# cts198859/deeprl_signal_control

Measured on NVIDIA H100. Metric: agent-env-steps/sec, higher is better.
Workload: dtype f32 (sim, LSTM cell, loss, optimizer) + bf16 tensor-core operands with f32 accumulation (learner GEMMs)

## Files before the change

### deeprl_signal_control_b200/_lib.py

```python
from __future__ import annotations

import ctypes as C
import os
import subprocess

_HERE = os.path.dirname(os.path.abspath(__file__))
CSRC = os.path.join(_HERE, "csrc")
LIB_PATH = os.environ.get("TSC_LIB", os.path.join(CSRC, "libtsc.so"))
_lib = None

SYMBOLS = ["tsc_last_error", "tsc_create", "tsc_destroy", "tsc_reset", "tsc_set_train_mode",
           "tsc_observe", "tsc_step", "tsc_step_host", "tsc_step_host_range", "tsc_step_host_range_async", "tsc_set_record", "tsc_step_record", "tsc_get_trips", "tsc_get_counts", "tsc_get_traffic_stats",
           "tsc_dump_state", "tsc_info", "tsc_mean_live", "tsc_set_greedy_program", "tsc_greedy_actions",
           "tscl_create", "tscl_destroy", "tscl_fc_embed", "tscl_lstm_seq_fwd", "tscl_heads", "tscl_returns",
           "tscl_heads_loss", "tscl_lstm_seq_bwd", "tscl_fc_bwd", "tscl_fc_bwd_tc", "tscl_wgrad_tc", "tscl_clip_rmsprop",
           "tscl_pack_weights", "tscl_policy_step", "tscl_policy_step_v2", "tscl_policy_step_v2r", "tscl_unpack_store", "tscl_pack_wht", "tscl_lstm_seq_bwd_tc", "tscl_pack_wxt", "tscl_lstm_seq_bwd_tc_dx", "tscl_dx_tc", "tscl_host_transition", "tscl_device_transition", "tscl_memcpy_async", "tscl_fc_hidden_fwd", "tscl_fc_hidden_bwd", "tscl_debug_policy_prof", "tscl_debug_bptt_prof",
           "tscl_policy_step_pi", "tscl_argmax_actions", "tscl_q_create", "tscl_q_destroy", "tscl_q_step",
           "tscl_q_explore", "tscl_q_sample", "tscl_q_td", "tscl_q_adam", "tscl_q_transition"]


def build_native(force: bool = False, verbose: bool = False) -> str:
    cmd = ["make", "-C", CSRC] + (["-B"] if force else [])
    out = subprocess.run(cmd, capture_output=True, text=True)
    if out.returncode != 0:
        raise RuntimeError("nvcc build of libtsc.so failed:\n" + out.stdout + out.stderr)
    if verbose:
        print(out.stdout + out.stderr)
    return LIB_PATH


def lib() -> C.CDLL:
    global _lib
    if _lib is None:
        if not os.path.exists(LIB_PATH):
            raise ImportError(
                "native library %s is missing: run `python -c 'import __graft_entry__ as g; g.build()'` "
                "(there is no CPU fallback)" % LIB_PATH)
        _lib = C.CDLL(LIB_PATH)
        _lib.tsc_last_error.restype = C.c_char_p
        for s in SYMBOLS:
            getattr(_lib, s)
    return _lib


def check(rc: int):
    if rc != 0:
        raise RuntimeError("libtsc: " + lib().tsc_last_error().decode())
```

### deeprl_signal_control_b200/agents/learner.py

```python
from __future__ import annotations

import ctypes as C
import os
from typing import Optional

import numpy as np
import torch

from .. import _lib
from .. import dist as _dist
from .layout import PolicyLayout


def _p(t):
    return None if t is None else C.c_void_p(t.data_ptr())


class BatchedA2C:
    def __init__(self, layout: PolicyLayout, n_replicas: int, n_step: int, gamma: float = 0.99,
                 v_coef: float = 0.5, max_grad_norm: float = 40.0, alpha: float = 0.99, eps: float = 1e-5,
                 reward_norm: float = 1.0, reward_clip: float = 0.0, seed: int = 0, device: int = 0,
                 chunk: int = 1024, replica0: int = 0, total_replicas: Optional[int] = None,
                 process_group=None, allow_tf32: bool = True, use_tc: bool = True,
                 store_acts: Optional[bool] = None):
# ... 27 lines not shown
        self.c_bw = torch.zeros_like(self.c_fw); self.h_bw = torch.zeros_like(self.h_fw)
        self.c_tmp = torch.zeros_like(self.c_fw); self.h_tmp = torch.zeros_like(self.h_fw)
        self.X1 = torch.empty(U, R, L.dx, **f32)
        self.Z1 = torch.empty(U, R, 4 * L.h, **f32)
        self.H1 = torch.empty(U, R, L.h, **f32)
        self.pi = torch.zeros(R, A, L.max_na, **f32)
        self.val = torch.zeros(R, A, **f32)
        self.act = torch.zeros(R, A, dtype=torch.int32, device=self.dev)
        self.boot = torch.zeros(R, A, **f32)
        self.obs_hist = torch.zeros(T + 1, R, L.n_obs, **f32)
        self.act_hist = torch.zeros(T, R, A, dtype=torch.int32, device=self.dev)
        self.rew_hist = torch.zeros(T, R, A, **f32)
        self.val_hist = torch.zeros(T, R, A, **f32)
        self.Rs = torch.zeros(T, R, A, **f32); self.Adv = torch.zeros(T, R, A, **f32)
        self.done_pre = [0.0] * T
        self.done_post = [0.0] * T
        self.last_done = False
        self.t = 0
        self.n_forward = 0
        self._one = torch.zeros(1, **f32)
        self._upd_bufs = None
        self.kernel_launches = 0
        self.use_tc = bool(use_tc) and (L.dx % 16 == 0) and layout.kw > 0
        if self.use_tc and L.dx > 224:
            raise ValueError("the tensor-core policy forward supports dx <= 224 (got %d); use use_tc=False" % L.dx)
        self.tc_v2 = self.use_tc and L.dx in (160, 192, 224)
        self.Wp = torch.zeros(U, ((L.dx + L.h) // 8) * 4 * L.h * 8 + 8 * L.dx * 8, dtype=torch.bfloat16,
                              device=self.dev)
        self.Wt = torch.zeros(U, 32, L.h, 8, dtype=torch.bfloat16, device=self.dev)
        self.Wxt = torch.zeros(U, 32, L.dx, 8, dtype=torch.bfloat16, device=self.dev)
        self.dx_fused = False
        self.dx_fusable = self.use_tc and L.dx % 32 == 0 and L.dx <= 256
        self.dx_own = self.use_tc and L.dx % 16 == 0 and L.dx <= 224 and os.environ.get("TSC_DX_LIBRARY", "0") != "1"
        self.bwd_tc = self.use_tc
        self.fc_bwd_tc = self.use_tc and layout.fc_bwd_tc_ok
        self.wgrad_tc = self.use_tc and L.dx % 8 == 0 and L.dx <= 240
        self.fused_heads = True
        self.pack_weights()
        need = U * T * R * (L.dx + 4 * L.h + 2 * L.h) * 2
        if store_acts is None:
            free, _ = torch.cuda.mem_get_info(self.dev)
            store_acts = self.tc_v2 and need < 0.5 * free
        self.store_acts = bool(store_acts) and self.tc_v2 and (R % self.chunk == 0)
        self.st_x = self.st_g = self.st_c = self.st_h = None
        if self.store_acts:
            bf = dict(dtype=torch.bfloat16, device=self.dev)
            nc, rc_ = R // self.chunk, self.chunk
            self.st_x = torch.zeros(nc, U, T, rc_, L.dx, **bf); self.st_g = torch.zeros(nc, U, T, rc_, 4 * L.h, **bf)
            self.st_c = torch.zeros(nc, U, T, rc_, L.h, **bf); self.st_h = torch.zeros(nc, U, T, rc_, L.h, **bf)
        self._acts_ok = [False] * T

    def close(self):
        if getattr(self, "_h", None) is not None:
            _lib.lib().tscl_destroy(self._h)
            self._h = None

    def __del__(self):
        try:
            self.close()
        except Exception:
            pass

    def _st(self):
        return C.c_void_p(torch.cuda.current_stream(self.dev).cuda_stream)

    def pack_weights(self):
# ... 97 lines not shown
        self.t += 1

    def obs_slot(self, t: Optional[int] = None) -> torch.Tensor:
        return self.obs_hist[self.t if t is None else t]

    def add_transition(self, reward: torch.Tensor, done_pre: bool, done_post: bool,
                       act: Optional[torch.Tensor] = None, val: Optional[torch.Tensor] = None):
        t = self.t
        r = reward
        if self.reward_norm:
            r = r / self.reward_norm
        if self.reward_clip:
            r = torch.clamp(r, -self.reward_clip, self.reward_clip)
        self.rew_hist[t].copy_(r)
        self.act_hist[t].copy_(self.act if act is None else act)
        self.val_hist[t].copy_(self.val if val is None else val)
        self.done_pre[t] = 1.0 if done_pre else 0.0
        self.done_post[t] = 1.0 if done_post else 0.0
        self.t += 1

    def add_transition_device(self, reward: torch.Tensor, greward: torch.Tensor, rew_acc: torch.Tensor, done_pre: bool,
                              done_post: bool):
        t = self.t
        _lib.check(_lib.lib().tscl_device_transition(
            self._h, _p(reward), _p(self.rew_hist[t]), C.c_int64(reward.numel()), C.c_float(self.reward_norm or 0.0),
            C.c_float(self.reward_clip or 0.0), _p(greward), _p(rew_acc), C.c_int64(greward.numel()), self._st()))
        if not getattr(self, "_hist_direct", False):
            self.act_hist[t].copy_(self.act)
            self.val_hist[t].copy_(self.val)
        self.done_pre[t] = 1.0 if done_pre else 0.0
        self.done_post[t] = 1.0 if done_post else 0.0
        self.t += 1

    def _bufs(self, rc, lean=False):
        L, T, U = self.lay, self.T, self.lay.U
        f32 = dict(dtype=torch.float32, device=self.dev)
        if self._upd_bufs is None or self._upd_bufs["rc"] < rc:
            M = T * rc
            self._upd_bufs = dict(rc=rc, dH=torch.empty(U, M, L.h, **f32))
        b = self._upd_bufs
        M = T * b["rc"]
        if lean and "dZb" not in b:
            b.update(dZb=torch.empty(U, M, 4 * L.h, dtype=torch.bfloat16, device=self.dev),
                     dXb=torch.empty(U, M, L.dx, dtype=torch.bfloat16, device=self.dev))
        if not lean and "X" not in b:
            b.update(ZG=torch.empty(U, M, 4 * L.h, **f32), dX=torch.empty(U, M, L.dx, **f32),
                     X=torch.empty(U, M, L.dx, **f32), C=torch.empty(U, M, L.h, **f32), H=torch.empty(U, M, L.h, **f32),
                     Hp=torch.empty(U, M, L.h, **f32), dlog=torch.empty(U, M, L.max_na, **f32))
        return b

    def backward(self, boot: Optional[torch.Tensor], lr: float, beta: float):
        assert self.t == self.T, "rollout buffer not full"
        L, R, T, U, A, lib = self.lay, self.R, self.T, self.lay.U, self.lay.A, _lib.lib()
        self._mm()
        st = self._st
        f32 = dict(dtype=torch.float32, device=self.dev)
        dpre = torch.tensor(self.done_pre, **f32)
        dpost = torch.tensor(self.done_post, **f32)
        if boot is None:
            self.boot.zero_()
        else:
            self.boot.copy_(boot)
        _lib.check(lib.tscl_returns(self._h, _p(self.rew_hist), _p(self.val_hist), _p(self.boot), _p(dpost),
                                    C.c_float(self.gamma), C.c_int32(T), C.c_int64(R), _p(self.Rs), _p(self.Adv), st()))
        self.G.zero_()
        self.stats.zero_()
        scale = _dist.grad_scale(T, 1, self.total_replicas)
        use_store = self.store_acts and all(self._acts_ok)
        n_obs = L.n_obs
        for r0 in range(0, R, self.chunk):
            rc = min(self.chunk, R - r0)
            M = T * rc
            ci = r0 // self.chunk
            all_tc = use_store and self.bwd_tc and self.fc_bwd_tc and self.wgrad_tc and self.fused_heads
            b = self._bufs(rc, lean=all_tc)
            X = Cc = H = Hp = dlog = ZG = dX = dZb = dXb = None
            bf16 = dict(dtype=torch.bfloat16, device=self.dev)
            if b["rc"] == rc:
                dH = b["dH"]
                if all_tc:
                    dZb, dXb = b["dZb"], b["dXb"]
                else:
                    ZG, dX, X, Cc, H, Hp, dlog = (b[k] for k in ("ZG", "dX", "X", "C", "H", "Hp", "dlog"))
            else:
                dH = torch.empty(U, M, L.h, **f32)
                if all_tc:
                    dZb, dXb = torch.empty(U, M, 4 * L.h, **bf16), torch.empty(U, M, L.dx, **bf16)
                else:
                    ZG, dX, X, Cc, H, Hp, dlog = (torch.empty(U, M, s_, **f32) for s_ in
                                                  (4 * L.h, L.dx, L.dx, L.h, L.h, L.h, L.max_na))
            obs0 = self.obs_hist[0, r0:]
            if all_tc:
                pass
            elif use_store:
                direct = self.bwd_tc
                _lib.check(lib.tscl_unpack_store(self._h, _p(self.st_x[ci]), _p(self.st_g[ci]), _p(self.st_c[ci]),
                                                 _p(self.st_h[ci]), _p(X), None if direct else _p(ZG),
                                                 None if direct else _p(Cc), _p(H), _p(Hp), _p(self.h_bw),
                                                 _p(dpre), C.c_int32(T), C.c_int64(rc), C.c_int64(R), C.c_int64(r0),
                                                 st()))
            else:
                _lib.check(lib.tscl_fc_embed(self._h, _p(self.P), _p(obs0), C.c_int64(M), C.c_int64(rc),
                                             C.c_int64(R * n_obs), _p(X), st()))
                torch.baddbmm(self.pv["bl"].unsqueeze(1), X, self.pv["wx"], out=ZG)
                _lib.check(lib.tscl_lstm_seq_fwd(self._h, _p(self.P), _p(ZG), _p(Cc), _p(H), _p(Hp), _p(self.c_bw),
                                                 _p(self.h_bw), None, None, _p(dpre), C.c_int32(T), C.c_int64(rc),
                                                 C.c_int64(R), C.c_int64(r0), st()))
            hb = _p(self.st_h[ci]) if use_store else None
            _lib.check(lib.tscl_heads_loss(self._h, _p(self.P), None if all_tc else _p(H), _p(self.act_hist[0, r0:]),
                                           _p(self.Rs[0, r0:]), _p(self.Adv[0, r0:]), C.c_int64(M), C.c_int64(rc),
                                           C.c_int64(R * A), C.c_float(self.v_coef), C.c_float(beta), C.c_float(scale),
                                           None if self.fused_heads else _p(dlog), _p(dH), _p(self.stats),
                                           hb if all_tc else None, _p(self.G) if self.fused_heads else None, st()))
            if not self.fused_heads:
                self.gv["wo"].baddbmm_(H.transpose(1, 2), dlog)
                self.gv["bo"].add_(dlog.sum(dim=1))
            fuse_dx = all_tc and self.dx_fused and self.dx_fusable
            if self.bwd_tc:
                gb = (_p(self.st_g[ci]), _p(self.st_c[ci])) if use_store else (None, None)
                _lib.check(lib.tscl_lstm_seq_bwd_tc_dx(self._h, _p(self.Wt), _p(ZG), _p(Cc), _p(dH), _p(self.c_bw),
                                                       _p(dpre), C.c_int32(T), C.c_int64(rc), C.c_int64(R), C.c_int64(r0),
                                                       *gb, _p(dZb), _p(self.Wxt) if fuse_dx else None,
                                                       _p(dXb) if fuse_dx else None, st()))
            else:
                _lib.check(lib.tscl_lstm_seq_bwd(self._h, _p(self.P), _p(ZG), _p(Cc), _p(dH), _p(self.c_bw), _p(dpre),
                                                 C.c_int32(T), C.c_int64(rc), C.c_int64(R), C.c_int64(r0), st()))
            dZ = ZG
            if self.wgrad_tc:
                if use_store:
                    _lib.check(lib.tscl_wgrad_tc(self._h, _p(dZ), _p(dZb), None, _p(self.st_x[ci]), None, _p(self.st_h[ci]),
                                                 _p(self.h_bw), _p(dpre), C.c_int32(T), C.c_int64(rc), C.c_int64(R),
                                                 C.c_int64(r0), _p(self.G), C.c_int32(0), st()))
                else:
                    _lib.check(lib.tscl_wgrad_tc(self._h, _p(dZ), None, _p(X), None, _p(Hp), None, None, None, C.c_int32(T),
                                                 C.c_int64(rc), C.c_int64(R), C.c_int64(r0), _p(self.G), C.c_int32(0), st()))
            else:
                self.gv["wx"].baddbmm_(X.transpose(1, 2), dZ)
                self.gv["wh"].baddbmm_(Hp.transpose(1, 2), dZ)
                self.gv["bl"].add_(dZ.sum(dim=1))
            if all_tc and not fuse_dx and self.dx_own:
                _lib.check(lib.tscl_dx_tc(self._h, _p(dZb), _p(self.Wxt), _p(dXb), C.c_int64(M), st()))
            elif all_tc and not fuse_dx:
                torch.bmm(dZb, self.wx_b.transpose(1, 2), out=dXb)
            elif not all_tc:
                torch.bmm(dZ, self.pv["wx"].transpose(1, 2), out=dX)
            if self.fc_bwd_tc:
                xb = _p(self.st_x[ci]) if use_store else None
                _lib.check(lib.tscl_fc_bwd_tc(self._h, _p(obs0), None if all_tc else _p(X), xb, _p(dX), _p(dXb),
                                              C.c_int64(M), C.c_int64(rc), C.c_int64(R * n_obs), _p(self.G), C.c_int32(0),
                                              st()))
            else:
                _lib.check(lib.tscl_fc_bwd(self._h, _p(obs0), _p(X), _p(dX), C.c_int64(M), C.c_int64(rc),
                                           C.c_int64(R * n_obs), _p(self.G), st()))
            self.kernel_launches += 4 if use_store else 5
        if self.pg is not None:
            _dist.allreduce_sum_(self.G, self.pg)
        _lib.check(lib.tscl_clip_rmsprop(self._h, _p(self.P), _p(self.G), _p(self.MS), _p(self.agent_of),
                                         C.c_float(self.max_grad_norm), C.c_float(lr), C.c_float(self.alpha),
                                         C.c_float(self.eps), _p(self.norms), st()))
        self.kernel_launches += 3
        self.pack_weights()
        self.c_bw.copy_(self.c_fw); self.h_bw.copy_(self.h_fw)
        self.obs_hist[0].copy_(self.obs_hist[T])
        self.last_done = bool(self.done_post[-1])
        self.t = 0
        self._acts_ok = [False] * T
```

### deeprl_signal_control_b200/csrc/tsc_policy_tc.cu

```cuda
#include <cuda.h>
#include <cstdlib>
#include <cuda_bf16.h>
#include <cuda_runtime.h>
#include <stdint.h>

#include <string>

#include "../../include/tsc_learn.h"

int tsc_set_error(const std::string& m);
#define PCK(call)                                                                  \
  do {                                                                             \
    cudaError_t e__ = (call);                                                      \
    if (e__ != cudaSuccess) return tsc_set_error(std::string(#call) + ": " + cudaGetErrorString(e__)); \
  } while (0)

struct DDimsTC {
  int A, n_obs, max_na, fw, ff, ft, h, dx;
  const int32_t *obs_off, *n_wave, *n_wait, *n_fp, *n_a;
  const int64_t *off_fcw_w, *off_fcw_b, *off_fcf_w, *off_fcf_b, *off_fct_w, *off_fct_b;
  int64_t off_wx, off_wh, off_bl, off_wo, off_bo, n_params;
  int kw, ones_slot;
};
const DDimsTC* tscl_dims_of(tscl_handle* h);
// ... 1363 lines not shown
      wg_fence();
#pragma unroll
      for (int g = 0; g < 4; ++g)
#pragma unroll
        for (int c = 0; c < 4; ++c)
          wgmma_n64_rs(acc, af[g][2 * c][0], af[g][2 * c][1], af[g][2 * c + 1][0], af[g][2 * c + 1][1],
                       make_desc(aB + (4 * g + c) * 2 * 1024, 1024, 128), (g | c) != 0);
      wg_commit();
      BR_MARK(2);
      asm volatile("bar.sync %0, 128;" ::"r"(1 + wg) : "memory");
      if (lead) {
#pragma unroll
        for (int g = 0; g < 4; ++g) tma_store_3d(&mapZ, g * 64, rw0, z0 + t, aZ + g * 8192);
        asm volatile("cp.async.bulk.commit_group;" ::: "memory");
      }
      BR_MARK(3);
      wg_wait<0>();
      wg_frag_fence(acc);
      const bool need_dh = keep != 0.f && t > 0;
#pragma unroll
      for (int j = 0; j < 8; ++j)
#pragma unroll
        for (int e = 0; e < 4; ++e) dhc[j][e] = need_dh ? acc[4 * j + e] * keep : 0.f;
      BR_MARK(2);
    }
  }
  if (lead) asm volatile("cp.async.bulk.wait_group 0;" ::: "memory");
  if (PROF && lead)
    for (int i = 0; i < 4; ++i) atomicAdd(a.prof + i, (unsigned long long)bp[i]);
#undef BR_MARK
}

static bool make_tmap_3d(CUtensorMap* m, CUtensorMapDataType dt, int elem_bytes, const void* base, uint64_t planes,
                         uint64_t rows, uint64_t cols, uint32_t box_cols, uint32_t box_rows) {
  typedef CUresult (*encode_fn)(CUtensorMap*, CUtensorMapDataType, cuuint32_t, void*, const cuuint64_t*, const cuuint64_t*,
                                const cuuint32_t*, const cuuint32_t*, CUtensorMapInterleave, CUtensorMapSwizzle,
                                CUtensorMapL2promotion, CUtensorMapFloatOOBfill);
  static encode_fn fn = []() -> encode_fn {
    void* p = nullptr;
    cudaDriverEntryPointQueryResult q;
    if (cudaGetDriverEntryPoint("cuTensorMapEncodeTiled", &p, cudaEnableDefault, &q) != cudaSuccess || q != cudaDriverEntryPointSuccess)
      return nullptr;
    return (encode_fn)p;
  }();
  if (!fn || !base) return false;
  memset(m, 0, sizeof(*m));
  const cuuint64_t dims[3] = {cols, rows, planes};
  const cuuint64_t strides[2] = {cols * (uint64_t)elem_bytes, rows * cols * (uint64_t)elem_bytes};
  const cuuint32_t box[3] = {box_cols, box_rows, 1};
  const cuuint32_t es[3] = {1, 1, 1};
  return fn(m, dt, 3, const_cast<void*>(base), dims, strides, box, es, CU_TENSOR_MAP_INTERLEAVE_NONE, CU_TENSOR_MAP_SWIZZLE_128B,
            CU_TENSOR_MAP_L2_PROMOTION_L2_128B, CU_TENSOR_MAP_FLOAT_OOB_FILL_NONE) == CUDA_SUCCESS;
}

__device__ __forceinline__ void cp_async16(uint32_t dst, const void* src) {
  asm volatile("cp.async.cg.shared.global [%0], [%1], 16;" ::"r"(dst), "l"(src) : "memory");
}

extern "C" int tscl_pack_wxt(tscl_handle* h, const float* params, void* wxt_bf16, void* stream) {
  if (!h || !params || !wxt_bf16) return tsc_set_error("tscl_pack_wxt: bad argument");
  PCK(cudaSetDevice(tscl_device_of(h)));
  const DDimsTC& d = *tscl_dims_of(h);
  pack_wxt_kernel<<<dim3(8, 2 * d.A), 256, 0, (cudaStream_t)stream>>>(d, params, (__nv_bfloat16*)wxt_bf16);
  PCK(cudaGetLastError());
  return 0;
}

extern "C" int tscl_pack_wht(tscl_handle* h, const float* params, void* wt_bf16, void* stream) {
  if (!h || !params || !wt_bf16) return tsc_set_error("tscl_pack_wht: bad argument");
  PCK(cudaSetDevice(tscl_device_of(h)));
  const DDimsTC& d = *tscl_dims_of(h);
  pack_wht_kernel<<<dim3(2, 2 * d.A), 256, 0, (cudaStream_t)stream>>>(d, params, (__nv_bfloat16*)wt_bf16);
  PCK(cudaGetLastError());
  return 0;
}

extern "C" int tscl_lstm_seq_bwd_tc(tscl_handle* h, const void* wt_bf16, float* ZG, const float* C, const float* dH,
                                    const float* c0, const float* done, int32_t T, int64_t Rc, int64_t ld_state,
                                    int64_t r0, const void* gates_bf16, const void* c_bf16, void* dz_bf16, void* stream) {
  return tscl_lstm_seq_bwd_tc_dx(h, wt_bf16, ZG, C, dH, c0, done, T, Rc, ld_state, r0, gates_bf16, c_bf16, dz_bf16, nullptr,
                                 nullptr, stream);
}

extern "C" int tscl_lstm_seq_bwd_tc_dx(tscl_handle* h, const void* wt_bf16, float* ZG, const float* C, const float* dH,
// ... 853 lines not shown
  __syncthreads();
}

extern "C" int tscl_dx_tc(tscl_handle* h, const void* dz_bf16, const void* wxt_bf16, void* dx_bf16, int64_t M, void* stream) {
  if (!h || !dz_bf16 || !wxt_bf16 || !dx_bf16 || M <= 0) return tsc_set_error("tscl_dx_tc: bad argument");
  PCK(cudaSetDevice(tscl_device_of(h)));
  const DDimsTC& d = *tscl_dims_of(h);
  if (d.dx % 16 != 0 || d.dx > 224 || d.dx < 16) return tsc_set_error("tscl_dx_tc: dx must be a multiple of 16 in [16, 224]");
  const size_t smem = (size_t)DXK_STAGES * DXK_STAGE_BYTES + (size_t)BW_KC * d.dx * 16 + (size_t)128 * (d.dx * 2 + 16) + 12 * 8 + 16;
  if (smem > 232448) return tsc_set_error("tscl_dx_tc: shared memory budget exceeded");
  void (*kern)(const DDimsTC, const DxTC) = nullptr;
  switch (d.dx) {
#define DXK_CASE(n) case n: kern = dx_tc_kernel<n>; break;
    DXK_CASE(16) DXK_CASE(32) DXK_CASE(48) DXK_CASE(64) DXK_CASE(80) DXK_CASE(96) DXK_CASE(112) DXK_CASE(128)
    DXK_CASE(144) DXK_CASE(160) DXK_CASE(176) DXK_CASE(192) DXK_CASE(208) DXK_CASE(224)
#undef DXK_CASE
  }
  static int attr_dev = -1;
  static void (*attr_kern)(const DDimsTC, const DxTC) = nullptr;
  if (attr_dev != tscl_device_of(h) || attr_kern != kern) {
    PCK(cudaFuncSetAttribute(kern, cudaFuncAttributeMaxDynamicSharedMemorySize, 232448));
    attr_dev = tscl_device_of(h); attr_kern = kern;
  }
  int n_sm = 0;
  PCK(cudaDeviceGetAttribute(&n_sm, cudaDevAttrMultiProcessorCount, tscl_device_of(h)));
  const int64_t NT = ((M + 127) / 128) * 2 * d.A;
  const int grid = (int)(NT < n_sm ? NT : n_sm);
  DxTC a;
  a.dZb = (const __nv_bfloat16*)dz_bf16; a.Wxt = (const __nv_bfloat16*)wxt_bf16; a.dXb = (__nv_bfloat16*)dx_bf16; a.M = M;
  kern<<<grid, DXK_THREADS, smem, (cudaStream_t)stream>>>(d, a);
  PCK(cudaGetLastError());
  return 0;
}
```

### include/tsc_learn.h

```cpp
#ifndef TSC_LEARN_H_
#define TSC_LEARN_H_

#include <stdint.h>

#ifdef __cplusplus
extern "C" {
#endif

typedef struct tscl_dims {
  int32_t n_agents;
  int32_t n_obs;
  int32_t max_na;
  int32_t fw, ff, ft;
  int32_t h;
  int32_t dx;
  const int32_t* obs_off;
  const int32_t* n_wave;
  const int32_t* n_wait;
  const int32_t* n_fp;
  const int32_t* n_a;
  const int64_t* off_fcw_w;  const int64_t* off_fcw_b;
  const int64_t* off_fcf_w;  const int64_t* off_fcf_b;
  const int64_t* off_fct_w;  const int64_t* off_fct_b;
  int64_t off_wx;
// ... 32 lines not shown
                    void* stream);

int tscl_lstm_seq_bwd(tscl_handle* h, const float* params, float* ZG, const float* C, const float* dH,
                      const float* c0, const float* done, int32_t T, int64_t Rc, int64_t ld_state, int64_t r0,
                      void* stream);

int tscl_fc_bwd(tscl_handle* h, const float* obs, const float* X, const float* dX, int64_t M,
                int64_t rows_per_t, int64_t stride_t, float* grads, void* stream);

int tscl_fc_bwd_tc(tscl_handle* h, const float* obs, const float* X, const void* x_bf16, const float* dX,
                   const void* dx_bf16, int64_t M, int64_t rows_per_t, int64_t stride_t, float* grads, int32_t variant,
                   void* stream);

int tscl_wgrad_tc(tscl_handle* h, const float* dZ, const void* dz_bf16, const float* X, const void* x_bf16,
                  const float* Hp, const void* h_bf16, const float* h0, const float* done, int32_t T, int64_t rc,
                  int64_t ld_state, int64_t r0, float* grads, int32_t variant, void* stream);

int tscl_pack_wht(tscl_handle* h, const float* params, void* wt_bf16, void* stream);
int tscl_lstm_seq_bwd_tc(tscl_handle* h, const void* wt_bf16, float* ZG, const float* C, const float* dH, const float* c0,
                         const float* done, int32_t T, int64_t Rc, int64_t ld_state, int64_t r0,
                         const void* gates_bf16, const void* c_bf16, void* dz_bf16, void* stream);
int tscl_pack_wxt(tscl_handle* h, const float* params, void* wxt_bf16, void* stream);
int tscl_lstm_seq_bwd_tc_dx(tscl_handle* h, const void* wt_bf16, float* ZG, const float* C, const float* dH, const float* c0,
                            const float* done, int32_t T, int64_t Rc, int64_t ld_state, int64_t r0,
                            const void* gates_bf16, const void* c_bf16, void* dz_bf16, const void* wxt_bf16, void* dx_bf16,
                            void* stream);
int tscl_host_transition(tscl_handle* h, const float* obs_host, float* obs_dev, int64_t obs_floats, const float* rew_host,
                         float* rew_stage_dev, float* rew_hist_dev, int64_t rew_floats, float reward_norm, float reward_clip,
                         const float* grew_host, float* grew_stage_dev, float* rew_acc_dev, int64_t n, void* stream);
int tscl_device_transition(tscl_handle* h, const float* rew_dev, float* rew_hist_dev, int64_t rew_floats, float reward_norm,
                           float reward_clip, const float* grew_dev, float* rew_acc_dev, int64_t n, void* stream);
int tscl_memcpy_async(tscl_handle* h, void* dst, const void* src, int64_t bytes, int32_t kind, void* stream);
int tscl_dx_tc(tscl_handle* h, const void* dz_bf16, const void* wxt_bf16, void* dx_bf16, int64_t M, void* stream);

int tscl_unpack_store(tscl_handle* h, const void* st_x, const void* st_g, const void* st_c, const void* st_h, float* X,
                      float* ZG, float* C, float* H, float* Hp, const float* h0, const float* done, int32_t T,
                      int64_t rc, int64_t ld_state, int64_t r0, void* stream);

int tscl_debug_policy_prof(void* counters_dev);
int tscl_debug_bptt_prof(void* counters_dev);

int tscl_clip_rmsprop(tscl_handle* h, float* params, float* grads, float* ms, const uint8_t* agent_of,
                      float max_norm, float lr, float alpha, float eps, float* norms, void* stream);

int tscl_pack_weights(tscl_handle* h, const float* params, void* wpack_bf16, void* stream);
int tscl_policy_step(tscl_handle* h, const float* params, const void* wpack_bf16, const float* obs, int64_t R,
                     const float* c_in, const float* h_in, float* c_out, float* h_out, float* pi, float* val,
                     int32_t* act, int32_t done, uint64_t seed, int64_t step, int64_t replica0, float* zdbg,
                     int32_t swap_lbo_sbo, void* stream);

int tscl_policy_step_v2(tscl_handle* h, const float* params, const void* wpack_bf16, const float* obs, int64_t R,
                        const float* c_in, const float* h_in, float* c_out, float* h_out, float* pi, float* val,
                        int32_t* act, int32_t done, uint64_t seed, int64_t step, int64_t replica0, float* zdbg,
                        void* st_x, void* st_g, void* st_c, void* st_h, int32_t t, int32_t T, int64_t rc, void* stream);
int tscl_policy_step_v2r(tscl_handle* h, const float* params, const void* wpack_bf16, const float* obs, int64_t R,
                         const float* c_in, const float* h_in, float* c_out, float* h_out, float* pi, float* val,
                         int32_t* act, int32_t done, uint64_t seed, int64_t step, int64_t replica0, float* zdbg,
                         void* st_x, void* st_g, void* st_c, void* st_h, int32_t t, int32_t T, int64_t rc,
                         int64_t ld_state, int64_t row0, void* stream);
int tscl_policy_step_pi(tscl_handle* h, const float* params, const void* wpack_bf16, const float* obs, int64_t R,
                        const float* c_in, const float* h_in, float* c_out, float* h_out, float* pi, int32_t* act,
                        int32_t act_mode, int32_t done, uint64_t seed, int64_t step, int64_t replica0, int64_t ld_state,
                        int64_t row0, void* stream);
int tscl_argmax_actions(tscl_handle* h, const float* pi, int64_t R, int32_t* act, void* stream);

typedef struct tscl_qdims {
// ... 40 lines not shown
```

Baseline: 22.59 million.

## Fuse LSTM input-gradient GEMM with FC-embedding weight-gradient backward kernel

Adds a warp-specialized Hopper kernel that computes dX = dZ·Wx^T with wgmma. It applies the ReLU mask from the stored activations in shared memory and immediately uses the masked dX tile for the FC weight-gradient GEMM against observations gathered on the fly. This removes the bf16 dX round trip through global memory and one kernel launch per chunk. In exchange it brings register-split setmaxnreg, TMA pipelines and atomic gradient flushes, limited to dx in {160,192,224}.

```diff
diff --git a/deeprl_signal_control_b200/_lib.py b/deeprl_signal_control_b200/_lib.py
--- a/deeprl_signal_control_b200/_lib.py
+++ b/deeprl_signal_control_b200/_lib.py
@@ -14,7 +14,7 @@
            "tsc_dump_state", "tsc_info", "tsc_mean_live", "tsc_set_greedy_program", "tsc_greedy_actions",
            "tscl_create", "tscl_destroy", "tscl_fc_embed", "tscl_lstm_seq_fwd", "tscl_heads", "tscl_returns",
            "tscl_heads_loss", "tscl_lstm_seq_bwd", "tscl_fc_bwd", "tscl_fc_bwd_tc", "tscl_wgrad_tc", "tscl_clip_rmsprop",
-           "tscl_pack_weights", "tscl_policy_step", "tscl_policy_step_v2", "tscl_policy_step_v2r", "tscl_unpack_store", "tscl_pack_wht", "tscl_lstm_seq_bwd_tc", "tscl_pack_wxt", "tscl_lstm_seq_bwd_tc_dx", "tscl_dx_tc", "tscl_host_transition", "tscl_device_transition", "tscl_memcpy_async", "tscl_fc_hidden_fwd", "tscl_fc_hidden_bwd", "tscl_debug_policy_prof", "tscl_debug_bptt_prof",
+           "tscl_pack_weights", "tscl_policy_step", "tscl_policy_step_v2", "tscl_policy_step_v2r", "tscl_unpack_store", "tscl_pack_wht", "tscl_lstm_seq_bwd_tc", "tscl_pack_wxt", "tscl_lstm_seq_bwd_tc_dx", "tscl_dx_tc", "tscl_dx_fc_bwd_tc", "tscl_host_transition", "tscl_device_transition", "tscl_memcpy_async", "tscl_fc_hidden_fwd", "tscl_fc_hidden_bwd", "tscl_debug_policy_prof", "tscl_debug_bptt_prof",
            "tscl_policy_step_pi", "tscl_argmax_actions", "tscl_q_create", "tscl_q_destroy", "tscl_q_step",
            "tscl_q_explore", "tscl_q_sample", "tscl_q_td", "tscl_q_adam", "tscl_q_transition"]
 
diff --git a/deeprl_signal_control_b200/agents/learner.py b/deeprl_signal_control_b200/agents/learner.py
--- a/deeprl_signal_control_b200/agents/learner.py
+++ b/deeprl_signal_control_b200/agents/learner.py
@@ -83,6 +83,7 @@
         self.dx_fused = False
         self.dx_fusable = self.use_tc and L.dx % 32 == 0 and L.dx <= 256
         self.dx_own = self.use_tc and L.dx % 16 == 0 and L.dx <= 224 and os.environ.get("TSC_DX_LIBRARY", "0") != "1"
+        self.dx_fc_fused = self.dx_own and self.tc_v2
         self.bwd_tc = self.use_tc
         self.fc_bwd_tc = self.use_tc and layout.fc_bwd_tc_ok
         self.wgrad_tc = self.use_tc and L.dx % 8 == 0 and L.dx <= 240
@@ -246,7 +247,7 @@
         self.done_post[t] = 1.0 if done_post else 0.0
         self.t += 1
 
-    def _bufs(self, rc, lean=False):
+    def _bufs(self, rc, lean=False, dxb=True):
         L, T, U = self.lay, self.T, self.lay.U
         f32 = dict(dtype=torch.float32, device=self.dev)
         if self._upd_bufs is None or self._upd_bufs["rc"] < rc:
@@ -255,8 +256,9 @@
         b = self._upd_bufs
         M = T * b["rc"]
         if lean and "dZb" not in b:
-            b.update(dZb=torch.empty(U, M, 4 * L.h, dtype=torch.bfloat16, device=self.dev),
-                     dXb=torch.empty(U, M, L.dx, dtype=torch.bfloat16, device=self.dev))
+            b["dZb"] = torch.empty(U, M, 4 * L.h, dtype=torch.bfloat16, device=self.dev)
+        if lean and dxb and "dXb" not in b:
+            b["dXb"] = torch.empty(U, M, L.dx, dtype=torch.bfloat16, device=self.dev)
         if not lean and "X" not in b:
             b.update(ZG=torch.empty(U, M, 4 * L.h, **f32), dX=torch.empty(U, M, L.dx, **f32),
                      X=torch.empty(U, M, L.dx, **f32), C=torch.empty(U, M, L.h, **f32), H=torch.empty(U, M, L.h, **f32),
@@ -287,19 +289,22 @@
             M = T * rc
             ci = r0 // self.chunk
             all_tc = use_store and self.bwd_tc and self.fc_bwd_tc and self.wgrad_tc and self.fused_heads
-            b = self._bufs(rc, lean=all_tc)
+            fuse_dx = all_tc and self.dx_fused and self.dx_fusable
+            fuse_fc = all_tc and not fuse_dx and self.dx_fc_fused
+            b = self._bufs(rc, lean=all_tc, dxb=not fuse_fc)
             X = Cc = H = Hp = dlog = ZG = dX = dZb = dXb = None
             bf16 = dict(dtype=torch.bfloat16, device=self.dev)
             if b["rc"] == rc:
                 dH = b["dH"]
                 if all_tc:
-                    dZb, dXb = b["dZb"], b["dXb"]
+                    dZb, dXb = b["dZb"], b.get("dXb")
                 else:
                     ZG, dX, X, Cc, H, Hp, dlog = (b[k] for k in ("ZG", "dX", "X", "C", "H", "Hp", "dlog"))
             else:
                 dH = torch.empty(U, M, L.h, **f32)
                 if all_tc:
-                    dZb, dXb = torch.empty(U, M, 4 * L.h, **bf16), torch.empty(U, M, L.dx, **bf16)
+                    dZb = torch.empty(U, M, 4 * L.h, **bf16)
+                    dXb = None if fuse_fc else torch.empty(U, M, L.dx, **bf16)
                 else:
                     ZG, dX, X, Cc, H, Hp, dlog = (torch.empty(U, M, s_, **f32) for s_ in
                                                   (4 * L.h, L.dx, L.dx, L.h, L.h, L.h, L.max_na))
@@ -329,7 +334,6 @@
             if not self.fused_heads:
                 self.gv["wo"].baddbmm_(H.transpose(1, 2), dlog)
                 self.gv["bo"].add_(dlog.sum(dim=1))
-            fuse_dx = all_tc and self.dx_fused and self.dx_fusable
             if self.bwd_tc:
                 gb = (_p(self.st_g[ci]), _p(self.st_c[ci])) if use_store else (None, None)
                 _lib.check(lib.tscl_lstm_seq_bwd_tc_dx(self._h, _p(self.Wt), _p(ZG), _p(Cc), _p(dH), _p(self.c_bw),
@@ -352,13 +356,18 @@
                 self.gv["wx"].baddbmm_(X.transpose(1, 2), dZ)
                 self.gv["wh"].baddbmm_(Hp.transpose(1, 2), dZ)
                 self.gv["bl"].add_(dZ.sum(dim=1))
-            if all_tc and not fuse_dx and self.dx_own:
+            if fuse_fc:
+                _lib.check(lib.tscl_dx_fc_bwd_tc(self._h, _p(obs0), _p(self.st_x[ci]), _p(dZb), _p(self.Wxt), C.c_int64(M),
+                                                 C.c_int64(rc), C.c_int64(R * n_obs), _p(self.G), st()))
+            elif all_tc and not fuse_dx and self.dx_own:
                 _lib.check(lib.tscl_dx_tc(self._h, _p(dZb), _p(self.Wxt), _p(dXb), C.c_int64(M), st()))
             elif all_tc and not fuse_dx:
                 torch.bmm(dZb, self.wx_b.transpose(1, 2), out=dXb)
             elif not all_tc:
                 torch.bmm(dZ, self.pv["wx"].transpose(1, 2), out=dX)
-            if self.fc_bwd_tc:
+            if fuse_fc:
+                pass
+            elif self.fc_bwd_tc:
                 xb = _p(self.st_x[ci]) if use_store else None
                 _lib.check(lib.tscl_fc_bwd_tc(self._h, _p(obs0), None if all_tc else _p(X), xb, _p(dX), _p(dXb),
                                               C.c_int64(M), C.c_int64(rc), C.c_int64(R * n_obs), _p(self.G), C.c_int32(0),
@@ -366,7 +375,7 @@
             else:
                 _lib.check(lib.tscl_fc_bwd(self._h, _p(obs0), _p(X), _p(dX), C.c_int64(M), C.c_int64(rc),
                                            C.c_int64(R * n_obs), _p(self.G), st()))
-            self.kernel_launches += 4 if use_store else 5
+            self.kernel_launches += 3 if fuse_fc else 4 if use_store else 5
         if self.pg is not None:
             _dist.allreduce_sum_(self.G, self.pg)
         _lib.check(lib.tscl_clip_rmsprop(self._h, _p(self.P), _p(self.G), _p(self.MS), _p(self.agent_of),
diff --git a/deeprl_signal_control_b200/csrc/tsc_policy_tc.cu b/deeprl_signal_control_b200/csrc/tsc_policy_tc.cu
--- a/deeprl_signal_control_b200/csrc/tsc_policy_tc.cu
+++ b/deeprl_signal_control_b200/csrc/tsc_policy_tc.cu
@@ -1419,7 +1419,8 @@
 }
 
 static bool make_tmap_3d(CUtensorMap* m, CUtensorMapDataType dt, int elem_bytes, const void* base, uint64_t planes,
-                         uint64_t rows, uint64_t cols, uint32_t box_cols, uint32_t box_rows) {
+                         uint64_t rows, uint64_t cols, uint32_t box_cols, uint32_t box_rows,
+                         CUtensorMapSwizzle sw = CU_TENSOR_MAP_SWIZZLE_128B) {
   typedef CUresult (*encode_fn)(CUtensorMap*, CUtensorMapDataType, cuuint32_t, void*, const cuuint64_t*, const cuuint64_t*,
                                 const cuuint32_t*, const cuuint32_t*, CUtensorMapInterleave, CUtensorMapSwizzle,
                                 CUtensorMapL2promotion, CUtensorMapFloatOOBfill);
@@ -1436,7 +1437,7 @@
   const cuuint64_t strides[2] = {cols * (uint64_t)elem_bytes, rows * cols * (uint64_t)elem_bytes};
   const cuuint32_t box[3] = {box_cols, box_rows, 1};
   const cuuint32_t es[3] = {1, 1, 1};
-  return fn(m, dt, 3, const_cast<void*>(base), dims, strides, box, es, CU_TENSOR_MAP_INTERLEAVE_NONE, CU_TENSOR_MAP_SWIZZLE_128B,
+  return fn(m, dt, 3, const_cast<void*>(base), dims, strides, box, es, CU_TENSOR_MAP_INTERLEAVE_NONE, sw,
             CU_TENSOR_MAP_L2_PROMOTION_L2_128B, CU_TENSOR_MAP_FLOAT_OOB_FILL_NONE) == CUDA_SUCCESS;
 }
 
@@ -2356,3 +2357,321 @@
   PCK(cudaGetLastError());
   return 0;
 }
+
+#define DXF_THREADS 384
+#define DXF_STAGES 2
+#define DXF_SBO 2048
+#define DXF_BUILDERS 96
+#define DXF_CONS_REGS(dx) ((dx) > 192 ? 216 : 208)
+#define DXF_PROD_REGS(dx) ((dx) > 192 ? 72 : 80)
+static_assert(128 * DXF_PROD_REGS(224) + 256 * DXF_CONS_REGS(224) <= DXF_THREADS * 168 &&
+              128 * DXF_PROD_REGS(160) + 256 * DXF_CONS_REGS(160) <= DXF_THREADS * 168,
+              "setmaxnreg split exceeds the CTA's registers");
+static size_t dxf_smem(int dx) {
+  return (size_t)DXF_STAGES * DXK_STAGE_BYTES + (size_t)BW_KC * dx * 16 + (size_t)(dx / 8) * DXF_SBO + 8 * FBT_SBO + 8 * 8;
+}
+struct DxFcTC {
+  const float* obs;
+  const __nv_bfloat16* Wxt;
+  float* G;
+  int64_t M, rows_per_t, stride_t;
+};
+__device__ __forceinline__ uint32_t bf16x2_pos_mask(uint32_t x) {
+  const uint32_t nz = ((x & 0x7FFF7FFFu) + 0x7FFF7FFFu) & ~x & 0x80008000u;
+  return (nz >> 15) * 0xFFFFu;
+}
+template <int NR>
+__device__ __forceinline__ void dxf_flush(const DDimsTC& d, float* G, int u, const float (&f)[NR], int cb) {
+  const int lane = threadIdx.x & 31, w4 = (threadIdx.x >> 5) & 3, ag = u >> 1;
+  const int nw = d.n_wave[ag], nt = d.n_wait[ag], nf = d.ff > 0 ? d.n_fp[ag] : 0;
+#pragma unroll
+  for (int e = 0; e < NR; ++e) {
+    const int slot = 16 * w4 + (lane >> 2) + 8 * ((e >> 1) & 1);
+    const int c = cb + 8 * (e >> 2) + 2 * (lane & 3) + (e & 1);
+    int64_t wo, bo; int ld, cc, s0, n;
+    if (c < d.fw) { wo = d.off_fcw_w[u]; bo = d.off_fcw_b[u]; ld = d.fw; cc = c; s0 = 0; n = nw; }
+    else if (c < d.fw + d.ff) { wo = d.off_fcf_w[u]; bo = d.off_fcf_b[u]; ld = d.ff; cc = c - d.fw; s0 = d.kw; n = nf; }
+    else { wo = d.off_fct_w[u]; bo = d.off_fct_b[u]; ld = d.ft; cc = c - d.fw - d.ff; s0 = d.kw + TC_KF; n = nt; }
+    const int kin = slot - s0;
+    if (kin >= 0 && kin < n) atomicAdd(&G[wo + (int64_t)kin * ld + cc], f[e]);
+    if (slot == d.ones_slot) atomicAdd(&G[bo + cc], f[e]);
+  }
+}
+
+template <int DX>
+__global__ void __launch_bounds__(DXF_THREADS, 1)
+dx_fc_bwd_tc_kernel(const DDimsTC d, const DxFcTC a, const __grid_constant__ CUtensorMap mapZ,
+                    const __grid_constant__ CUtensorMap mapX) {
+  constexpr int N64 = DX / 64, R32 = (DX % 64) >= 32, R16 = (DX % 32) >= 16;
+  constexpr int HN = DX / 2, H32 = (HN % 64) >= 32, H16 = (HN % 32) >= 16;
+  static_assert(HN >= 64 && HN < 128 && HN % 16 == 0, "fc half width must be 64 + {0, 16, 32, 48}");
+  const int tid = threadIdx.x, warp = tid >> 5, lane = tid & 31;
+  unsigned char* sStage = tc_smem;
+  unsigned char* sW = sStage + DXF_STAGES * DXK_STAGE_BYTES;
+  unsigned char* sA = sW + (size_t)BW_KC * DX * 16;
+  unsigned char* sB = sA + (size_t)(DX / 8) * DXF_SBO;
+  uint64_t* sBar = reinterpret_cast<uint64_t*>(sB + 8 * FBT_SBO);
+  const uint32_t bar_full = smem_u32(sBar), bar_empty = bar_full + 16, bar_w = bar_full + 32, bar_x = bar_full + 40,
+                 bar_in = bar_full + 48, bar_free = bar_full + 56;
+  if (tid == 0) {
+    for (int s = 0; s < DXF_STAGES; ++s) { mbar_init(bar_full + 8 * s, 1); mbar_init(bar_empty + 8 * s, 8); }
+    mbar_init(bar_w, 1); mbar_init(bar_x, 1); mbar_init(bar_in, DXF_BUILDERS); mbar_init(bar_free, 8);
+    asm volatile("fence.mbarrier_init.release.cluster;" ::: "memory");
+  }
+  __syncthreads();
+#define DXF_RANGE                                                                                   \
+  const int64_t tpu = (a.M + 127) / 128;                                                            \
+  const int64_t NT = tpu * 2 * d.A;                                                                 \
+  const int64_t j0 = NT * blockIdx.x / gridDim.x, j1 = NT * (blockIdx.x + 1) / gridDim.x;
+
+  if (warp >= 8) {
+    asm volatile("setmaxnreg.dec.sync.aligned.u32 %0;" ::"n"(DXF_PROD_REGS(DX)));
+    DXF_RANGE
+    if (warp == 8) {
+      if (lane == 0) {
+        const uint32_t aS = smem_u32(sStage), aA = smem_u32(sA);
+        int64_t it = 0;
+        for (int64_t j = j0; j < j1; ++j) {
+          const int u = (int)(j / tpu), m0 = (int)((j - (int64_t)u * tpu) * 128);
+          auto atom = [&](int at) {
+            const int s = (int)(it % DXF_STAGES);
+            const int64_t n = it / DXF_STAGES;
+            if (n > 0) mbar_wait(bar_empty + 8 * s, (uint32_t)((n - 1) & 1));
+            mbar_expect_tx(bar_full + 8 * s, DXK_STAGE_BYTES);
+            tma_load_3d(aS + s * DXK_STAGE_BYTES, &mapZ, at * 64, m0, u, bar_full + 8 * s);
+            ++it;
+          };
+          atom(0); atom(1);
+          if (j > j0) mbar_wait(bar_free, (uint32_t)((j - j0 - 1) & 1));
+          mbar_expect_tx(bar_x, (DX / 8) * DXF_SBO);
+#pragma unroll 1
+          for (int cg = 0; cg < DX / 8; ++cg) tma_load_3d(aA + cg * DXF_SBO, &mapX, cg * 8, m0, u, bar_x);
+          atom(2); atom(3);
+        }
+      }
+    } else {
+      const int bt = tid - 288, bc = bt & 7;
+      int cur_u = -1, ooff = 0;
+      int src[8];
+      for (int64_t j = j0; j < j1; ++j) {
+        const int u = (int)(j / tpu);
+        const int64_t m0 = (j - (int64_t)u * tpu) * 128;
+        if (u != cur_u) {
+          cur_u = u;
+          const int ag = u >> 1;
+          const int nw = d.n_wave[ag], nt = d.n_wait[ag], nf = d.ff > 0 ? d.n_fp[ag] : 0;
+          ooff = d.obs_off[ag];
+#pragma unroll
+          for (int e = 0; e < 8; ++e) {
+            const int slot = bc * 8 + e;
+            int sidx = -1;
+            if (slot < d.kw) { if (slot < nw) sidx = slot; }
+            else if (slot < d.kw + TC_KF) { if (slot - d.kw < nf) sidx = nw + nt + (slot - d.kw); }
+            else { if (slot - d.kw - TC_KF < nt) sidx = nw + (slot - d.kw - TC_KF); }
+            if (slot == d.ones_slot) sidx = -2;
+            src[e] = sidx;
+          }
+        }
+        const int rows_valid = (a.M - m0) < 128 ? (int)(a.M - m0) : 128;
+        const int64_t tq = m0 / a.rows_per_t, rem0 = m0 - tq * a.rows_per_t;
+        if (j > j0) mbar_wait(bar_free, (uint32_t)((j - j0 - 1) & 1));
+#pragma unroll 1
+        for (int i = bt; i < 128 * 8; i += 2 * DXF_BUILDERS) {
+          float v[2][8];
+#pragma unroll
+          for (int p = 0; p < 2; ++p) {
+            const int row = (i + p * DXF_BUILDERS) >> 3;
+#pragma unroll
+            for (int e = 0; e < 8; ++e) v[p][e] = 0.f;
+            if (i + p * DXF_BUILDERS < 128 * 8 && row < rows_valid) {
+              int64_t tt = tq, rem = rem0 + row;
+              while (rem >= a.rows_per_t) { rem -= a.rows_per_t; ++tt; }
+              const float* op = a.obs + tt * a.stride_t + rem * d.n_obs + ooff;
+#pragma unroll
+              for (int e = 0; e < 8; ++e) v[p][e] = src[e] >= 0 ? __ldg(op + src[e]) : (src[e] == -2 ? 1.0f : 0.f);
+            }
+          }
+#pragma unroll
+          for (int p = 0; p < 2; ++p) {
+            const int ii = i + p * DXF_BUILDERS;
+            if (ii < 128 * 8) {
+              __align__(16) __nv_bfloat16 o[8];
+#pragma unroll
+              for (int e = 0; e < 8; ++e) o[e] = __float2bfloat16_rn(v[p][e]);
+              *reinterpret_cast<uint4*>(sB + (size_t)bc * FBT_SBO + (ii >> 3) * 16) = *reinterpret_cast<const uint4*>(o);
+            }
+          }
+        }
+        asm volatile("fence.proxy.async.shared::cta;" ::: "memory");
+        mbar_arrive(bar_in);
+        if (j + 1 < j1) {
+          const int un = (int)((j + 1) / tpu);
+          const int ooff_n = d.obs_off[un >> 1];
+          for (int r = bt; r < 128; r += DXF_BUILDERS) {
+            const int64_t m = (j + 1 - (int64_t)un * tpu) * 128 + r;
+            if (m >= a.M) break;
+            const float* op = a.obs + (m / a.rows_per_t) * a.stride_t + (m % a.rows_per_t) * d.n_obs + ooff_n;
+            asm volatile("prefetch.global.L2 [%0];" ::"l"(op));
+            asm volatile("prefetch.global.L2 [%0];" ::"l"(op + 32));
+          }
+        }
+      }
+    }
+  } else {
+    asm volatile("setmaxnreg.inc.sync.aligned.u32 %0;" ::"n"(DXF_CONS_REGS(DX)));
+    DXF_RANGE
+    const int wg = warp >> 2;
+    const uint32_t aS = smem_u32(sStage), aW = smem_u32(sW), aA = smem_u32(sA), aB = smem_u32(sB);
+    const uint32_t b_lbo = (uint32_t)DX * 16;
+    float f64[N64][32], f32[R32 ? 16 : 1], f16[R16 ? 8 : 1];
+    float g64[32], g32[H32 ? 16 : 1], g16[H16 ? 8 : 1];
+    const int n0 = wg * HN;
+    int64_t it = 0;
+    int cur_u = -1, prev_s = 0;
+    uint32_t wph = 0;
+    bool first = true;
+    const int fr = wg * 64 + (warp & 3) * 16 + (lane >> 2), c0 = 2 * (lane & 3);
+    auto mask_put = [&](int col, float x, float y, int r) {
+      uint32_t* p = reinterpret_cast<uint32_t*>(sA + (size_t)(col >> 3) * DXF_SBO + r * 16 + (col & 7) * 2);
+      const __nv_bfloat162 v = __floats2bfloat162_rn(x, y);
+      *p = *reinterpret_cast<const uint32_t*>(&v) & bf16x2_pos_mask(*p);
+    };
+    auto flush = [&](int u) {
+      dxf_flush(d, a.G, u, g64, n0);
+      if constexpr (H32) dxf_flush(d, a.G, u, g32, n0 + 64);
+      if constexpr (H16) dxf_flush(d, a.G, u, g16, n0 + 64 + 32 * H32);
+    };
+    for (int64_t j = j0; j < j1; ++j) {
+      const int u = (int)(j / tpu);
+      const uint32_t ph = (uint32_t)((j - j0) & 1);
+      if (u != cur_u) {
+        if (cur_u >= 0) flush(cur_u);
+        cur_u = u; first = true;
+        asm volatile("bar.sync 1, 256;" ::: "memory");
+        if (tid == 0) {
+          const uint32_t bytes = (uint32_t)BW_KC * DX * 16;
+          mbar_expect_tx(bar_w, bytes);
+          bulk_g2s(aW, a.Wxt + (int64_t)u * BW_KC * DX * 8, bytes, bar_w);
+        }
+        mbar_wait(bar_w, wph); wph ^= 1;
+      }
+      for (int at = 0; at < 4; ++at, ++it) {
+        const int s = (int)(it % DXF_STAGES);
+        mbar_wait(bar_full + 8 * s, (uint32_t)((it / DXF_STAGES) & 1));
+        const uint32_t a0 = aS + s * DXK_STAGE_BYTES + wg * 8192;
+        const uint32_t b0 = aW + (uint32_t)(at * 8) * b_lbo;
+        wg_fence();
+#pragma unroll
+        for (int q = 0; q < N64; ++q)
+          wg_mma_regs<64, 0, 0>(f64[q], 4, at > 0, [&](int k, uint64_t& da, uint64_t& db) {
+            da = make_desc_sw128(a0 + k * 32);
+            db = make_desc(b0 + (uint32_t)(k * 2) * b_lbo + q * 64 * 16, b_lbo, 128);
+          });
+        if constexpr (R32)
+          wg_mma_regs<32, 0, 0>(f32, 4, at > 0, [&](int k, uint64_t& da, uint64_t& db) {
+            da = make_desc_sw128(a0 + k * 32);
+            db = make_desc(b0 + (uint32_t)(k * 2) * b_lbo + N64 * 64 * 16, b_lbo, 128);
+          });
+        if constexpr (R16)
+          wg_mma_regs<16, 0, 0>(f16, 4, at > 0, [&](int k, uint64_t& da, uint64_t& db) {
+            da = make_desc_sw128(a0 + k * 32);
+            db = make_desc(b0 + (uint32_t)(k * 2) * b_lbo + (N64 * 64 + R32 * 32) * 16, b_lbo, 128);
+          });
+        wg_commit();
+        if (at > 0) {
+          wg_wait<1>();
+          if (lane == 0) mbar_arrive(bar_empty + 8 * prev_s);
+        }
+        prev_s = s;
+      }
+      wg_wait<0>();
+      if (lane == 0) mbar_arrive(bar_empty + 8 * prev_s);
+#pragma unroll
+      for (int q = 0; q < N64; ++q) wg_frag_fence(f64[q]);
+      if constexpr (R32) wg_frag_fence(f32);
+      if constexpr (R16) wg_frag_fence(f16);
+      mbar_wait(bar_x, ph);
+#pragma unroll
+      for (int q = 0; q < N64; ++q)
+#pragma unroll
+        for (int i = 0; i < 8; ++i) {
+          mask_put(q * 64 + 8 * i + c0, f64[q][4 * i], f64[q][4 * i + 1], fr);
+          mask_put(q * 64 + 8 * i + c0, f64[q][4 * i + 2], f64[q][4 * i + 3], fr + 8);
+        }
+      if constexpr (R32)
+#pragma unroll
+        for (int i = 0; i < 4; ++i) {
+          mask_put(N64 * 64 + 8 * i + c0, f32[4 * i], f32[4 * i + 1], fr);
+          mask_put(N64 * 64 + 8 * i + c0, f32[4 * i + 2], f32[4 * i + 3], fr + 8);
+        }
+      if constexpr (R16)
+#pragma unroll
+        for (int i = 0; i < 2; ++i) {
+          mask_put(N64 * 64 + R32 * 32 + 8 * i + c0, f16[4 * i], f16[4 * i + 1], fr);
+          mask_put(N64 * 64 + R32 * 32 + 8 * i + c0, f16[4 * i + 2], f16[4 * i + 3], fr + 8);
+        }
+      mbar_wait(bar_in, ph);
+      asm volatile("fence.proxy.async.shared::cta;" ::: "memory");
+      asm volatile("bar.sync 1, 256;" ::: "memory");
+      wg_fence();
+      wg_mma_regs<64, 1, 1>(g64, 8, !first, [&](int ks, uint64_t& da, uint64_t& db) {
+        da = make_desc(aB + ks * 256, 128, FBT_SBO);
+        db = make_desc(aA + (n0 / 8) * DXF_SBO + ks * 256, 128, DXF_SBO);
+      });
+      if constexpr (H32)
+        wg_mma_regs<32, 1, 1>(g32, 8, !first, [&](int ks, uint64_t& da, uint64_t& db) {
+          da = make_desc(aB + ks * 256, 128, FBT_SBO);
+          db = make_desc(aA + ((n0 + 64) / 8) * DXF_SBO + ks * 256, 128, DXF_SBO);
+        });
+      if constexpr (H16)
+        wg_mma_regs<16, 1, 1>(g16, 8, !first, [&](int ks, uint64_t& da, uint64_t& db) {
+          da = make_desc(aB + ks * 256, 128, FBT_SBO);
+          db = make_desc(aA + ((n0 + 64 + 32 * H32) / 8) * DXF_SBO + ks * 256, 128, DXF_SBO);
+        });
+      wg_commit();
+      wg_wait<0>();
+      wg_frag_fence(g64);
+      if constexpr (H32) wg_frag_fence(g32);
+      if constexpr (H16) wg_frag_fence(g16);
+      if (lane == 0) mbar_arrive(bar_free);
+      first = false;
+    }
+    if (cur_u >= 0) flush(cur_u);
+  }
+#undef DXF_RANGE
+}
+
+extern "C" int tscl_dx_fc_bwd_tc(tscl_handle* h, const float* obs, const void* x_bf16, const void* dz_bf16,
+                                 const void* wxt_bf16, int64_t M, int64_t rows_per_t, int64_t stride_t, float* grads,
+                                 void* stream) {
+  if (!h || !obs || !x_bf16 || !dz_bf16 || !wxt_bf16 || !grads || M <= 0 || rows_per_t <= 0)
+    return tsc_set_error("tscl_dx_fc_bwd_tc: bad argument");
+  if (M >= ((int64_t)1 << 31) - 128) return tsc_set_error("tscl_dx_fc_bwd_tc: M must be below 2^31 - 128 rows");
+  PCK(cudaSetDevice(tscl_device_of(h)));
+  const DDimsTC& d = *tscl_dims_of(h);
+  if (!P2_DX_OK(d.dx)) return tsc_set_error("tscl_dx_fc_bwd_tc: dx must be 160, 192 or 224 (use tscl_dx_tc + tscl_fc_bwd_tc)");
+  if (d.kw == 0 || d.ones_slot < 0) return tsc_set_error("tscl_dx_fc_bwd_tc: no free input slot for the bias column");
+  CUtensorMap mZ, mX;
+  if (!make_tmap_3d(&mZ, CU_TENSOR_MAP_DATA_TYPE_BFLOAT16, 2, dz_bf16, 2 * d.A, M, TC_N, 64, 128) ||
+      !make_tmap_3d(&mX, CU_TENSOR_MAP_DATA_TYPE_BFLOAT16, 2, x_bf16, 2 * d.A, M, d.dx, 8, 128, CU_TENSOR_MAP_SWIZZLE_NONE))
+    return tsc_set_error("tscl_dx_fc_bwd_tc: cannot build the tensor maps (dz_bf16 / x_bf16 must be 16-byte aligned)");
+  void (*kern)(const DDimsTC, const DxFcTC, const CUtensorMap, const CUtensorMap) =
+      d.dx == 224 ? dx_fc_bwd_tc_kernel<224> : d.dx == 192 ? dx_fc_bwd_tc_kernel<192> : dx_fc_bwd_tc_kernel<160>;
+  const size_t smem = dxf_smem(d.dx);
+  static int attr_dev = -1;
+  if (attr_dev != tscl_device_of(h)) {
+    PCK(cudaFuncSetAttribute(dx_fc_bwd_tc_kernel<224>, cudaFuncAttributeMaxDynamicSharedMemorySize, (int)dxf_smem(224)));
+    PCK(cudaFuncSetAttribute(dx_fc_bwd_tc_kernel<192>, cudaFuncAttributeMaxDynamicSharedMemorySize, (int)dxf_smem(192)));
+    PCK(cudaFuncSetAttribute(dx_fc_bwd_tc_kernel<160>, cudaFuncAttributeMaxDynamicSharedMemorySize, (int)dxf_smem(160)));
+    attr_dev = tscl_device_of(h);
+  }
+  int n_sm = 0;
+  PCK(cudaDeviceGetAttribute(&n_sm, cudaDevAttrMultiProcessorCount, tscl_device_of(h)));
+  const int64_t NT = ((M + 127) / 128) * 2 * d.A;
+  const int grid = (int)(NT < n_sm ? NT : n_sm);
+  DxFcTC a;
+  a.obs = obs; a.Wxt = (const __nv_bfloat16*)wxt_bf16; a.G = grads; a.M = M; a.rows_per_t = rows_per_t; a.stride_t = stride_t;
+  kern<<<grid, DXF_THREADS, smem, (cudaStream_t)stream>>>(d, a, mZ, mX);
+  PCK(cudaGetLastError());
+  return 0;
+}
diff --git a/include/tsc_learn.h b/include/tsc_learn.h
--- a/include/tsc_learn.h
+++ b/include/tsc_learn.h
@@ -88,6 +88,8 @@
                            float reward_clip, const float* grew_dev, float* rew_acc_dev, int64_t n, void* stream);
 int tscl_memcpy_async(tscl_handle* h, void* dst, const void* src, int64_t bytes, int32_t kind, void* stream);
 int tscl_dx_tc(tscl_handle* h, const void* dz_bf16, const void* wxt_bf16, void* dx_bf16, int64_t M, void* stream);
+int tscl_dx_fc_bwd_tc(tscl_handle* h, const float* obs, const void* x_bf16, const void* dz_bf16, const void* wxt_bf16,
+                      int64_t M, int64_t rows_per_t, int64_t stride_t, float* grads, void* stream);
 
 int tscl_unpack_store(tscl_handle* h, const void* st_x, const void* st_g, const void* st_c, const void* st_h, float* X,
                       float* ZG, float* C, float* H, float* Hp, const float* h0, const float* done, int32_t T,
```

Measured after the change: 26.19 million (median of 6 runs). 1.16x the previous value.
